# openfheorg/openfhe-development

Measured on AMD Instinct MI355X. Metric: NTT GB/s vs HBM roofline + CKKS EvalMultKeySwitch/sec, N=2^16 L=30, 1/2/4/8 GPU, higher is better.
Workload: dtype u64; 1 GPU; batched fwd+inv negacyclic NTT, N=2^16, L=30 x 60-bit limbs, 1024 polynomials per GPU (BASELINE configs[1]); global_batch=1024, parallelism=batch-sharded x1, no data-path collective

## Files before the change

openfhe-development_amd/csrc/fhe_hip.cpp:

```cpp
#include "../../include/fhe_hip.h"

#include <algorithm>
#include <cmath>
#include <cstdio>
#include <cstdlib>
#include <map>
#include <mutex>
#include <shared_mutex>
#include <string>
#include <type_traits>
#include <vector>

#include "basis_kernels.h"
#include "bfv_kernels.h"
#include "elemwise_kernels.h"
#include "host_math.h"
#include "ntt_kernels.h"
#include "ntt_static.h"
#include "ntt_row8.h"
#include "rt.h"
#include "sampler_kernels.h"
#include "blake2_kernels.h"

using namespace fhe;

static thread_local std::string g_lastError;
static fhe_status fail(fhe_status code, const std::string& msg) {
    g_lastError = msg;
    return code;
}
#define RT_CHECK(expr)                                                                  \
    do {                                                                                \
        const char* _e = (expr);                                                        \
        if (_e)                                                                         \
            return fail(FHE_ERR_DEVICE, std::string(#expr) + ": " + _e);                \
    } while (0)
#define ARG_CHECK(cond, msg)                  \
    do {                                      \
        if (!(cond))                          \
            return fail(FHE_ERR_ARG, msg);    \
    } while (0)

extern "C" const char* fhe_last_error(void) { return g_lastError.c_str(); }
extern "C" const char* fhe_version(void) {
#ifdef FHE_EMU
    return "fhe_hip 0.1 (TEST lane emulator build — not a product build)";
#else
    return "fhe_hip 0.1 (gfx950)";
#endif
}
extern "C" int fhe_device_count(void) { return rt::device_count(); }

namespace fhe {
namespace host {
bool is_prime(uint64_t n) {
    static const uint64_t w[] = {2, 3, 5, 7, 11, 13, 17, 19, 23, 29, 31, 37};
    if (n < 2)
        return false;
    for (uint64_t p : w) {
        if (n == p)
            return true;
        if (n % p == 0)
            return false;
    }
    uint64_t d = n - 1;
    int s      = 0;
    while (!(d & 1)) {
        d >>= 1;
        ++s;
    }
    for (uint64_t a : w) {
        uint64_t x = powmod(a, d, n);
        if (x == 1 || x == n - 1)
            continue;
        bool comp = true;
        for (int r = 1; r < s && comp; ++r) {
            x = mulmod(x, x, n);
            if (x == n - 1)
                comp = false;
        }
        if (comp)
            return false;
    }
    return true;
}
bool is_primitive_root_2n(uint64_t psi, uint64_t twoN, uint64_t q) {
    return psi != 0 && psi < q && powmod(psi, twoN / 2, q) == q - 1;
}
uint64_t first_prime(uint32_t bits, uint64_t m) {
    uint64_t q = (uint64_t)1 << bits, r = q % m, c = q + 1 - r;
    if (r > 0)
        c += m;
    while (!is_prime(c))
        c += m;
    return c;
}
uint64_t last_prime(uint32_t bits, uint64_t m) {
// ... 328 lines not shown
extern "C" fhe_status fhe_event_create(fhe_ctx* c, void** event) {
    ARG_CHECK(c && event, "fhe_event_create: null argument");
    RT_CHECK(rt::set_device(c->device));
    rt::event_t e;
    RT_CHECK(rt::event_create(&e));
    *event = (void*)e;
    return FHE_OK;
}
extern "C" fhe_status fhe_event_record(fhe_ctx* c, void* event, void* stream) {
    ARG_CHECK(c && event, "fhe_event_record: null argument");
    RT_CHECK(rt::set_device(c->device));
    RT_CHECK(rt::event_record((rt::event_t)event, (rt::stream_t)stream));
    return FHE_OK;
}
extern "C" fhe_status fhe_stream_wait_event(fhe_ctx* c, void* stream, void* event) {
    ARG_CHECK(c && event, "fhe_stream_wait_event: null argument");
    RT_CHECK(rt::set_device(c->device));
    RT_CHECK(rt::stream_wait_event((rt::stream_t)stream, (rt::event_t)event));
    return FHE_OK;
}
extern "C" fhe_status fhe_event_destroy(fhe_ctx* c, void* event) {
    ARG_CHECK(c, "fhe_event_destroy: null context");
    if (event)
        RT_CHECK(rt::event_destroy((rt::event_t)event));
    return FHE_OK;
}
extern "C" fhe_status fhe_memset_zero(fhe_ctx* c, void* dst, size_t bytes, void* stream) {
    ARG_CHECK(c && dst, "fhe_memset_zero: null argument");
    RT_CHECK(rt::set_device(c->device));
    RT_CHECK(rt::dzero(dst, bytes, (rt::stream_t)stream));
    return FHE_OK;
}
extern "C" fhe_status fhe_graph_begin(fhe_ctx* c, void* stream) {
    ARG_CHECK(c && stream, "fhe_graph_begin: capture needs a stream created with fhe_stream_create");
    RT_CHECK(rt::set_device(c->device));
    RT_CHECK(rt::capture_begin((rt::stream_t)stream));
    return FHE_OK;
}
extern "C" fhe_status fhe_graph_end(fhe_ctx* c, void* stream, void** graph) {
    ARG_CHECK(c && stream && graph, "fhe_graph_end: null argument");
    rt::graph_t g;
    RT_CHECK(rt::capture_end((rt::stream_t)stream, &g));
    *graph = (void*)g;
    return FHE_OK;
}
extern "C" fhe_status fhe_graph_launch(fhe_ctx* c, void* graph, void* stream) {
    ARG_CHECK(c && graph, "fhe_graph_launch: null argument");
    RT_CHECK(rt::graph_launch((rt::graph_t)graph, (rt::stream_t)stream));
    return FHE_OK;
}
extern "C" void fhe_graph_destroy(void* graph) {
    if (graph)
        rt::graph_destroy((rt::graph_t)graph);
}

static fhe_status make_sel(const fhe_ctx* c, const uint32_t* limbIdx, uint32_t nLimbs, LimbSel* sel, const char* who) {
    if (nLimbs < 1 || nLimbs > (uint32_t)kMaxLimbs)
        return fail(FHE_ERR_ARG, std::string(who) + ": nLimbs out of range");
    for (uint32_t i = 0; i < nLimbs; ++i) {
        uint32_t l = limbIdx ? limbIdx[i] : i;
        if (l >= c->L)
            return fail(FHE_ERR_ARG, std::string(who) + ": limb index exceeds context size");
        sel->idx[i] = (uint8_t)l;
    }
    for (uint32_t i = nLimbs; i < (uint32_t)kMaxLimbs; ++i)
        sel->idx[i] = 0;
    return FHE_OK;
}
static inline uint32_t tiles_for(const fhe_ctx* c, uint64_t rows) {
    const uint64_t words = rows << c->logN;
    return (uint32_t)((words + kTile - 1) >> kTileLog);
}
#define LAUNCH_CHECK() RT_CHECK(rt::last_launch_error())

static uint32_t env_u32(const char* name, uint32_t dflt) {
    const char* v = std::getenv(name);
    return v ? (uint32_t)std::strtoul(v, nullptr, 10) : dflt;
}
constexpr bool kHandoverDefault = true;
struct NttSwitches {
    int row8 = -1, row8X1 = -1;
    uint32_t row8Batch = 0, t1 = 0;
    bool handover = kHandoverDefault;
};
static const NttSwitches& ntt_switches() {
    static const NttSwitches sw = [] {
        NttSwitches s;
        auto flag = [](const char* name) {
            const char* v = std::getenv(name);
            return v && (v[0] == '0' || v[0] == '1') ? v[0] - '0' : -1;
        };
        s.row8   = flag("FHE_NTT_ROW8");
        s.row8X1 = flag("FHE_NTT_ROW8_X1");
        if (const char* v = std::getenv("FHE_NTT_ROW8_BATCH"))
            s.row8Batch = (v[0] == '1' || v[0] == '2' || v[0] == '4') && !v[1] ? (uint32_t)(v[0] - '0') : 0u;
        if (const char* v = std::getenv("FHE_NTT_HANDOVER")) {
            s.handover = v[0] == '1' && !v[1];
            if (!s.handover && !(v[0] == '0' && !v[1]))
                fprintf(stderr, "fhe_hip: FHE_NTT_HANDOVER=%s is neither 0 nor 1: hand-over is off\n", v);
        }
        s.t1 = env_u32("FHE_NTT_T1", 0);
        return s;
    }();
    return sw;
}
static bool row8_for(uint32_t T) { return ntt_switches().row8 >= 0 ? ntt_switches().row8 == 1 : T <= 11u; }
constexpr uint32_t kRow8BatchDefault = 2;
constexpr bool kRow8X1RegionsP2 = false, kRow8X1RegionsP4 = false;
static uint32_t row8_batch_for(uint32_t T) {
    if (T != 12u)
        return 1u;
    return ntt_switches().row8Batch ? ntt_switches().row8Batch : ntt_switches().row8 >= 0 ? 1u : kRow8BatchDefault;
}
static bool row8_x1_regions(uint32_t P) {
    return ntt_switches().row8X1 >= 0 ? ntt_switches().row8X1 == 1 : (P == 2 ? kRow8X1RegionsP2 : kRow8X1RegionsP4);
}
static uint32_t ntt_t1(uint32_t logN) {
    const uint32_t forced = ntt_switches().t1;
    if (forced >= 4 && forced <= 5 && logN > (uint32_t)kTileLog && logN - forced >= 9 && logN - forced <= 12)
        return forced;
    return std::max(4u, logN - (uint32_t)kTileLog);
}

struct NttPass {
    enum Kind { Single, Column, Row };
    bool inverse = false;
    Kind kind    = Single;
    uint32_t T   = 0;
    int mode = 1;
    NttPass() = default;
    NttPass(bool inv, Kind k, uint32_t stages) : inverse(inv), kind(k), T(stages), mode(k == Row ? (inv ? 0 : 9) : 1) {}
    bool layoutA() const { return kind == Column; }
};
struct NttPasses {
    uint32_t n;
    NttPass p[2];
};
static NttPasses ntt_passes(const fhe_ctx* c, bool inverse) {
    if (c->logN <= (uint32_t)kTileLog)
        return {1, {NttPass(inverse, NttPass::Single, c->logN), NttPass()}};
    const uint32_t T1 = ntt_t1(c->logN);
    const NttPass col(inverse, NttPass::Column, T1), row(inverse, NttPass::Row, c->logN - T1);
    return inverse ? NttPasses{2, {row, col}} : NttPasses{2, {col, row}};
}

struct NttEpilogue {
    uint32_t mode = 0, split = 0, aStride = 0, aFirst = 0;
    int64_t aDelta = 0;
    const uint64_t* A = nullptr;
    const TwPair* C   = nullptr;
    uint64_t *out0 = nullptr, *out1 = nullptr;
};
struct NttView {
    uint32_t stride = 0;
    uint32_t first  = 0;
};
struct NttOpts {
    NttView src, dst;
    int64_t srcDelta = 0;
    const NttEpilogue* epi = nullptr;
    bool canonOut = true;
    const uint32_t* proSrcLimb = nullptr;
    const TwPair* proC = nullptr;
    uint32_t proRows = 0;
};

static void plan_pass(bool inverse, bool layoutA, NttPassArgs& a) {
    const uint32_t logN = a.logN, T = a.T;
    const int logC  = kTileLog - (int)T;
    const int jsh   = layoutA ? (int)(logN - T) : 0;
    const int ish   = layoutA ? logC : 0;
    const int nst   = (int)(T + 3) / 4;
    int sizes[4];
    for (int i = 0; i < nst; ++i)
        sizes[i] = (int)T / nst + (i < (int)T % nst ? 1 : 0);
    NttStep real[4] = {};
// ... 798 lines not shown
    a.out = out, a.q = c->d_q, a.logN = c->logN, a.nLimbs = nl, a.batch = bt, a.seed = seed, a.stream = streamId, a.kind = kind;
    a.cdf = nullptr, a.cdfLen = 0, a.a = 0.0;
    if (kind == 1)
        if (fhe_status s = dgg_table(c, sigma, &a.cdf, &a.cdfLen, &a.a, who))
            return s;
    const uint64_t lanes = kind == 0 ? ((uint64_t)bt * nl) << c->logN : (uint64_t)bt << c->logN;
    FHE_LAUNCH(sample_kernel, (uint32_t)((lanes + kThreads - 1) / kThreads), st, a);
    LAUNCH_CHECK();
    return FHE_OK;
}
extern "C" fhe_status fhe_sample_uniform(fhe_ctx* c, uint64_t* out, const uint32_t* li, uint32_t nl, uint32_t bt, uint64_t seed,
                                         uint32_t streamId, void* st) {
    return sample_run(c, out, li, nl, bt, 0, 0.0, seed, streamId, st, "fhe_sample_uniform");
}
extern "C" fhe_status fhe_sample_gaussian(fhe_ctx* c, uint64_t* out, const uint32_t* li, uint32_t nl, uint32_t bt, double sigma,
                                          uint64_t seed, uint32_t streamId, void* st) {
    return sample_run(c, out, li, nl, bt, 1, sigma, seed, streamId, st, "fhe_sample_gaussian");
}
extern "C" fhe_status fhe_sample_ternary(fhe_ctx* c, uint64_t* out, const uint32_t* li, uint32_t nl, uint32_t bt, uint64_t seed,
                                         uint32_t streamId, void* st) {
    return sample_run(c, out, li, nl, bt, 2, 0.0, seed, streamId, st, "fhe_sample_ternary");
}

template <int KIND>
static fhe_status blake2_launch(const fhe_ctx* c, Blake2Args& a, const uint32_t* key, uint64_t counter0, void* st) {
    for (int i = 0; i < 16; ++i)
        a.key[i] = key[i];
    a.counter0 = counter0;
    const uint64_t minWaves = 8ull * (c->cus ? c->cus : 256);
    a.walk = kB2MaxWalk;
    while (a.walk > 1 && a.nBlocks / a.walk < minWaves)
        a.walk >>= 1;
    const uint64_t perWg = (uint64_t)(kB2Threads / 64) * a.walk;
    if (a.nBlocks)
        FHE_LAUNCH_BARRIER_N(blake2xb_kernel<KIND>, (a.nBlocks + perWg - 1) / perWg, kB2Threads, st, a);
    for (int i = 0; i < 16; ++i)
        ((volatile uint32_t*)a.key)[i] = 0;
    LAUNCH_CHECK();
    return FHE_OK;
}
extern "C" fhe_status fhe_blake2xb_stream(fhe_ctx* c, uint32_t* out, uint64_t nBlocks, const uint32_t key[16], uint64_t counter0, void* st) {
    ARG_CHECK(c && key && (out || nBlocks == 0), "fhe_blake2xb_stream: null argument");
    ARG_CHECK(((uintptr_t)out & 7u) == 0, "fhe_blake2xb_stream: out must be 8-byte aligned");
    ARG_CHECK(nBlocks <= ((uint64_t)UINT32_MAX - 1) * 4, "fhe_blake2xb_stream: nBlocks too large for one launch");
    RT_CHECK(rt::set_device(c->device));
    Blake2Args a{};
    a.out = (uint64_t*)out, a.nBlocks = nBlocks;
    return blake2_launch<3>(c, a, key, counter0, st);
}
static fhe_status blake2_sample(fhe_ctx* c, uint64_t* out, const uint32_t* li, uint32_t nl, uint32_t bt, int kind, double sigma,
                                const uint32_t* key, uint64_t counter0, void* st, const char* who) {
    ARG_CHECK(c && out && key && bt >= 1, std::string(who) + ": null argument or empty batch");
    Blake2Args a{};
    if (fhe_status s = make_sel(c, li, nl, &a.sel, who))
        return s;
    RT_CHECK(rt::set_device(c->device));
    a.out = out, a.q = c->d_q, a.mu128 = c->d_mu128, a.logN = c->logN, a.nLimbs = nl;
    if (kind == 1)
        if (fhe_status s = dgg_table(c, sigma, &a.cdf, &a.cdfLen, &a.a, who))
            return s;
    a.total   = kind == 0 ? ((uint64_t)bt * nl) << c->logN : (uint64_t)bt << c->logN;
    a.nBlocks = kind == 0 ? (a.total + 255) / 256 : (a.total + 511) / 512;
    return kind == 0   ? blake2_launch<0>(c, a, key, counter0, st)
           : kind == 1 ? blake2_launch<1>(c, a, key, counter0, st)
                       : blake2_launch<2>(c, a, key, counter0, st);
}
extern "C" fhe_status fhe_sample_uniform_blake2(fhe_ctx* c, uint64_t* out, const uint32_t* li, uint32_t nl, uint32_t bt,
                                                const uint32_t key[16], uint64_t counter0, void* st) {
    return blake2_sample(c, out, li, nl, bt, 0, 0.0, key, counter0, st, "fhe_sample_uniform_blake2");
}
extern "C" fhe_status fhe_sample_gaussian_blake2(fhe_ctx* c, uint64_t* out, const uint32_t* li, uint32_t nl, uint32_t bt, double sigma,
                                                 const uint32_t key[16], uint64_t counter0, void* st) {
    return blake2_sample(c, out, li, nl, bt, 1, sigma, key, counter0, st, "fhe_sample_gaussian_blake2");
}
extern "C" fhe_status fhe_sample_ternary_blake2(fhe_ctx* c, uint64_t* out, const uint32_t* li, uint32_t nl, uint32_t bt,
                                                const uint32_t key[16], uint64_t counter0, void* st) {
    return blake2_sample(c, out, li, nl, bt, 2, 0.0, key, counter0, st, "fhe_sample_ternary_blake2");
}

struct fhe_conv {
    fhe_ctx* ctx;
    uint32_t nSrc, nDst;
    std::vector<uint32_t> srcIdx, dstIdx;
    ConvTables tb;
    std::vector<ConvTables> chunks;
    const TwPair* allHatInv  = nullptr;
    const uint64_t* allSrcQ  = nullptr;
    const double* allQInv    = nullptr;
    std::vector<void*> owned;
};

static uint32_t conv_nsrc_pad(uint32_t nSrc) { return nSrc <= 8 ? 8u : nSrc <= 16 ? 16u : 32u; }
static fhe_status conv_from_tables(fhe_ctx* c, const std::vector<uint64_t>& src, const std::vector<uint64_t>& dst,
                                   const uint64_t* hatInvIn, const uint64_t* hatModIn, const uint64_t* alphaIn,
                                   const double* qInvIn, fhe_conv** out) {
    const uint32_t nSrc = (uint32_t)src.size(), nDst = (uint32_t)dst.size();
    if (nSrc < 1 || nSrc > (uint32_t)kMaxLimbs || nDst < 1 || nDst > (uint32_t)kMaxLimbs)
        return fail(FHE_ERR_ARG, "basis conversion: 1..256 source and target limbs");
    fhe_conv* cv = new fhe_conv;
    cv->ctx      = c;
    cv->nSrc     = nSrc;
    cv->nDst     = nDst;
    std::vector<uint64_t> mu(2 * (size_t)nDst), alphaMod((size_t)(nSrc + 1) * nDst, 0), red(4 * (size_t)nDst);
    for (uint32_t j = 0; j < nDst; ++j) {
        host::mu128(dst[j], &mu[2 * j]);
        const uint64_t R = (uint64_t)((((unsigned __int128)1) << 64) % dst[j]);
        red[4 * j]       = dst[j];
        red[4 * j + 1]   = R;
        red[4 * j + 2]   = host::shoup(R, dst[j]);
        red[4 * j + 3]   = (uint64_t)((((unsigned __int128)1) << 64) / dst[j]);
    }
    if (alphaIn)
        for (size_t k = 0; k < alphaMod.size(); ++k)
            alphaMod[k] = alphaIn[k] % dst[k % nDst];
    ConvTables shared{};
    fhe_status s;
    if ((s = dev_copy(&cv->owned, dst.data(), dst.size(), &shared.dstQ)) ||
        (s = dev_copy(&cv->owned, mu.data(), mu.size(), &shared.dstMu)) ||
        (s = dev_copy(&cv->owned, red.data(), red.size(), &shared.dstRed)) ||
        (s = dev_copy(&cv->owned, alphaMod.data(), alphaMod.size(), &shared.alphaMod))) {
        fhe_conv_destroy(cv);
        return s;
    }
    for (uint32_t c0 = 0; c0 < nSrc; c0 += 32u) {
        const uint32_t n   = std::min(32u, nSrc - c0);
        const uint32_t pad = conv_nsrc_pad(n);
        std::vector<TwPair> hatInv(32, TwPair{0, 0});
        std::vector<uint64_t> hatMod((size_t)pad * nDst, 0), srcPad(32, 1);
        std::vector<double> qInv(32, 0.0);
        for (uint32_t i = 0; i < n; ++i) {
            const uint64_t inv = hatInvIn[c0 + i] % src[c0 + i];
            hatInv[i]          = TwPair{inv, host::shoup(inv, src[c0 + i])};
            qInv[i]            = qInvIn ? qInvIn[c0 + i] : 1.0 / static_cast<double>(src[c0 + i]);
            srcPad[i]          = src[c0 + i];
            for (uint32_t j = 0; j < nDst; ++j)
                hatMod[(size_t)j * pad + i] = hatModIn[(size_t)(c0 + i) * nDst + j] % dst[j];
        }
        ConvTables tb = shared;
        if ((s = dev_copy(&cv->owned, hatInv.data(), hatInv.size(), &tb.hatInv)) ||
            (s = dev_copy(&cv->owned, hatMod.data(), hatMod.size(), &tb.hatMod)) ||
            (s = dev_copy(&cv->owned, srcPad.data(), srcPad.size(), &tb.srcQ)) ||
            (s = dev_copy(&cv->owned, qInv.data(), qInv.size(), &tb.srcQInv))) {
            fhe_conv_destroy(cv);
            return s;
        }
        cv->chunks.push_back(tb);
    }
    cv->tb = cv->chunks[0];
    if (nSrc > 32u) {
        std::vector<TwPair> allInv(nSrc);
        std::vector<double> allQInv(nSrc);
        for (uint32_t i = 0; i < nSrc; ++i) {
            const uint64_t inv = hatInvIn[i] % src[i];
            allInv[i]          = TwPair{inv, host::shoup(inv, src[i])};
            allQInv[i]         = qInvIn ? qInvIn[i] : 1.0 / static_cast<double>(src[i]);
        }
        if ((s = dev_copy(&cv->owned, allInv.data(), allInv.size(), &cv->allHatInv)) ||
            (s = dev_copy(&cv->owned, src.data(), src.size(), &cv->allSrcQ)) ||
            (s = dev_copy(&cv->owned, allQInv.data(), allQInv.size(), &cv->allQInv))) {
            fhe_conv_destroy(cv);
            return s;
        }
    }
    *out = cv;
    return FHE_OK;
}
static fhe_status conv_build(fhe_ctx* c, const std::vector<uint64_t>& src, const std::vector<uint64_t>& dst, fhe_conv** out,
                             const uint64_t* srcScale = nullptr, const uint64_t* dstScale = nullptr) {
    const uint32_t nSrc = (uint32_t)src.size(), nDst = (uint32_t)dst.size();
    std::vector<uint64_t> hatInv(nSrc), hatMod((size_t)nSrc * nDst), alphaMod((size_t)(nSrc + 1) * nDst);
    for (uint32_t i = 0; i < nSrc; ++i) {
        const uint64_t hat = host::prod_mod(src, (int)i, src[i]);
        hatInv[i]          = host::invmod(hat, src[i]);
        if (srcScale)
            hatInv[i] = host::mulmod(hatInv[i], srcScale[i] % src[i], src[i]);
        for (uint32_t j = 0; j < nDst; ++j) {
            uint64_t v = host::prod_mod(src, (int)i, dst[j]);
            if (dstScale)
                v = host::mulmod(v, dstScale[j] % dst[j], dst[j]);
            hatMod[(size_t)i * nDst + j] = v;
        }
    }
    for (uint32_t j = 0; j < nDst; ++j) {
        const uint64_t Qmod = host::prod_mod(src, -1, dst[j]);
        for (uint32_t a = 0; a <= nSrc; ++a)
// ... 31 lines not shown
    std::vector<uint64_t> src(nSrc), dst(nDst);
    for (uint32_t i = 0; i < nSrc; ++i) {
        ARG_CHECK(srcIdx[i] < c->L, "fhe_conv_create_custom: source limb exceeds context size");
        src[i] = c->q[srcIdx[i]];
    }
    for (uint32_t j = 0; j < nDst; ++j) {
        ARG_CHECK(dstIdx[j] < c->L, "fhe_conv_create_custom: target limb exceeds context size");
        dst[j] = c->q[dstIdx[j]];
    }
    RT_CHECK(rt::set_device(c->device));
    if (fhe_status s = conv_from_tables(c, src, dst, hatInv, hatMod, alphaMod, qInv, out))
        return s;
    (*out)->srcIdx.assign(srcIdx, srcIdx + nSrc);
    (*out)->dstIdx.assign(dstIdx, dstIdx + nDst);
    return FHE_OK;
}
extern "C" void fhe_conv_destroy(fhe_conv* cv) {
    if (!cv)
        return;
    for (void* p : cv->owned)
        rt::dfree(p);
    delete cv;
}

template <bool EXACT>
static fhe_status conv_run(fhe_conv* cv, const uint64_t* in, uint32_t inStride, uint32_t inFirst, uint64_t* out,
                           uint32_t outStride, uint32_t outFirst, uint32_t batch, void* st) {
    ARG_CHECK(cv && in && out, "fhe_switch_basis: null argument");
    ARG_CHECK(batch >= 1 && inFirst + cv->nSrc <= inStride && outFirst + cv->nDst <= outStride,
              "fhe_switch_basis: limb window exceeds tower stride");
    RT_CHECK(rt::set_device(cv->ctx->device));
    ConvArgs g{};
    g.in = in, g.out = out, g.tb = cv->tb;
    g.logN = cv->ctx->logN, g.batch = batch, g.nSrc = cv->nSrc, g.nDst = cv->nDst;
    g.inStride = inStride, g.inFirst = inFirst, g.outStride = outStride, g.outFirst = outFirst;
    const uint64_t coeffs = (uint64_t)batch << g.logN;
    const uint32_t grid   = (uint32_t)((coeffs + kThreads - 1) / kThreads);
    static const bool split30 = env_u32("FHE_CONV_SUM8", 2) != 1u;
    if (cv->chunks.size() > 1) {
        g.nSrcAll = cv->nSrc, g.inAll = in + ((size_t)inFirst << g.logN);
        g.allHatInv = cv->allHatInv, g.allSrcQ = cv->allSrcQ, g.allQInv = cv->allQInv;
        for (size_t k = 0; k < cv->chunks.size(); ++k) {
            g.tb      = cv->chunks[k];
            g.nSrc    = std::min(32u, cv->nSrc - 32u * (uint32_t)k);
            g.inFirst = inFirst + 32u * (uint32_t)k;
            g.acc     = k > 0;
            g.last    = k + 1 == cv->chunks.size();
            const uint32_t pad = conv_nsrc_pad(g.nSrc);
            if (pad == 8)
                FHE_LAUNCH((switch_basis_kernel<8, EXACT, 2, true>), grid, st, g);
            else if (pad == 16)
                FHE_LAUNCH((switch_basis_kernel<16, EXACT, 2, true>), grid, st, g);
            else
                FHE_LAUNCH((switch_basis_kernel<32, EXACT, 2, true>), grid, st, g);
            LAUNCH_CHECK();
        }
        return FHE_OK;
    }
    const uint32_t pad = conv_nsrc_pad(cv->nSrc);
    if (pad == 8 && split30)
        FHE_LAUNCH((switch_basis_kernel<8, EXACT, 2>), grid, st, g);
    else if (pad == 8)
        FHE_LAUNCH((switch_basis_kernel<8, EXACT, 1>), grid, st, g);
    else if (pad == 16 && split30)
        FHE_LAUNCH((switch_basis_kernel<16, EXACT, 2>), grid, st, g);
    else if (pad == 16)
        FHE_LAUNCH((switch_basis_kernel<16, EXACT, 1>), grid, st, g);
    else if (split30)
        FHE_LAUNCH((switch_basis_kernel<32, EXACT, 2>), grid, st, g);
    else
        FHE_LAUNCH((switch_basis_kernel<32, EXACT, 1>), grid, st, g);
    LAUNCH_CHECK();
    return FHE_OK;
}
extern "C" fhe_status fhe_approx_switch_basis(fhe_conv* cv, const uint64_t* in, uint32_t is, uint32_t ifst,
                                              uint64_t* out, uint32_t os, uint32_t ofst, uint32_t b, void* st) {
    return conv_run<false>(cv, in, is, ifst, out, os, ofst, b, st);
}
extern "C" fhe_status fhe_switch_basis_exact(fhe_conv* cv, const uint64_t* in, uint32_t is, uint32_t ifst,
                                             uint64_t* out, uint32_t os, uint32_t ofst, uint32_t b, void* st) {
    return conv_run<true>(cv, in, is, ifst, out, os, ofst, b, st);
}

extern "C" size_t fhe_expand_crt_basis_workspace_bytes(const fhe_conv* cv, uint32_t batch) {
    return cv ? (((size_t)batch * cv->nSrc) << cv->ctx->logN) * 8 : 0;
}
static fhe_status expand_run(fhe_conv* cv, const uint64_t* x, int inEval, uint64_t* out, int resultEval, int reverseOrder,
                             uint32_t batch, void* ws, size_t wsBytes, void* st, bool exact) {
    ARG_CHECK(cv && x && out && batch >= 1, "fhe_expand_crt_basis: bad argument");
    ARG_CHECK(!cv->srcIdx.empty(), "fhe_expand_crt_basis: the plan must come from fhe_conv_create[_custom]");
    fhe_ctx* c = cv->ctx;
    RT_CHECK(rt::set_device(c->device));
    const uint32_t nQ = cv->nSrc, nP = cv->nDst, tot = nQ + nP;
    const uint32_t qFirst = reverseOrder ? nP : 0, pFirst = reverseOrder ? 0 : nQ;
    const size_t rowB = (size_t)8 << c->logN;
    const uint64_t* coef = x;
    if (inEval) {
        ARG_CHECK(ws && wsBytes >= fhe_expand_crt_basis_workspace_bytes(cv, batch), "fhe_expand_crt_basis: workspace too small");
        if (fhe_status s = ntt_run(c, true, x, (uint64_t*)ws, cv->srcIdx.data(), nQ, batch, st))
            return s;
        coef = (const uint64_t*)ws;
    }
    if (fhe_status s = exact ? conv_run<true>(cv, coef, nQ, 0, out, tot, pFirst, batch, st)
                             : conv_run<false>(cv, coef, nQ, 0, out, tot, pFirst, batch, st))
        return s;
    const uint64_t* qsrc = (resultEval && inEval) ? x : coef;
    uint64_t* qdst       = out + ((size_t)qFirst << c->logN);
    RT_CHECK(rt::d2d_2d(qdst, tot * rowB, qsrc, nQ * rowB, nQ * rowB, batch, (rt::stream_t)st));
    if (resultEval) {
        NttOpts rows;
        rows.src.stride = rows.dst.stride = tot;
        rows.src.first = rows.dst.first = qFirst;
        if (!inEval)
            if (fhe_status s = ntt_run(c, false, out, out, cv->srcIdx.data(), nQ, batch, st, rows))
                return s;
        rows.src.first = rows.dst.first = pFirst;
        return ntt_run(c, false, out, out, cv->dstIdx.data(), nP, batch, st, rows);
    }
    return FHE_OK;
}
extern "C" fhe_status fhe_expand_crt_basis(fhe_conv* cv, const uint64_t* x, int inEval, uint64_t* out, int resultEval,
                                           int reverseOrder, uint32_t batch, void* ws, size_t wsBytes, void* st) {
    return expand_run(cv, x, inEval, out, resultEval, reverseOrder, batch, ws, wsBytes, st, true);
}
extern "C" fhe_status fhe_mod_up(fhe_conv* cv, const uint64_t* x, int inEval, uint64_t* out, uint32_t batch, void* ws,
                                 size_t wsBytes, void* st) {
    return expand_run(cv, x, inEval, out, 1, 0, batch, ws, wsBytes, st, false);
}
extern "C" fhe_status fhe_fast_expand_crt_basis_p_over_q(fhe_conv* toPl, fhe_conv* toQl, const uint64_t* x, uint64_t* out,
                                                         uint32_t batch, void* st) {
    ARG_CHECK(toPl && toQl && x && out && batch >= 1, "fhe_fast_expand_crt_basis_p_over_q: bad argument");
    ARG_CHECK(toQl->nSrc == toPl->nDst, "fhe_fast_expand_crt_basis_p_over_q: the second plan must start from the first plan's target basis");
    const uint32_t nQl = toQl->nDst, nPl = toPl->nDst, tot = nQl + nPl;
    if (fhe_status s = conv_run<false>(toPl, x, toPl->nSrc, 0, out, tot, nQl, batch, st))
        return s;
    return conv_run<true>(toQl, out, tot, nQl, out, tot, 0, batch, st);
}

struct fhe_ks_plan {
    fhe_ctx* ctx;
    uint32_t sizeQ, sizeP, numPartQ, alpha;
    struct Level {
        uint32_t sizeQl = 0, numParts = 0;
        std::vector<fhe_conv*> up;
        std::vector<std::vector<uint32_t>> cidx;
        std::vector<uint32_t> partSize;
        fhe_conv* down = nullptr;
        std::map<uint64_t, fhe_conv*> downT;
        TwPair* d_PInv = nullptr;
        TwPair* d_PModq = nullptr;
    };
    std::vector<Level*> levels;
    std::vector<void*> owned;
    std::map<std::vector<uint64_t>, void*> bsgsTables;
    uint64_t* d_zeroRows = nullptr;
    std::mutex cacheMutex;
};
struct fhe_ks_key {
    fhe_ks_plan* plan;
    uint64_t *d_b = nullptr, *d_a = nullptr;
    size_t words = 0;
    bool owned = true;
};

extern "C" fhe_status fhe_ks_plan_create(fhe_ctx* c, uint32_t sizeQ, uint32_t sizeP, uint32_t numPartQ,
                                         fhe_ks_plan** out) {
    ARG_CHECK(c && out, "fhe_ks_plan_create: null argument");
    ARG_CHECK(sizeQ >= 1 && sizeP >= 1 && sizeQ + sizeP <= c->L, "fhe_ks_plan_create: context must hold Q then P limbs");
    ARG_CHECK(numPartQ >= 1, "numPartQ is zero");
    const uint32_t a = (sizeQ + numPartQ - 1) / numPartQ;
    ARG_CHECK(sizeQ > a * (numPartQ - 1),
              "HYBRID key switching parameters: Can't appropriately distribute towers into digits");
    fhe_ks_plan* p = new fhe_ks_plan;
    p->ctx = c, p->sizeQ = sizeQ, p->sizeP = sizeP, p->numPartQ = numPartQ, p->alpha = a;
    p->levels.assign(sizeQ + 1, nullptr);
    *out = p;
    return FHE_OK;
}
static void ks_level_free(fhe_ks_plan::Level* lv) {
    if (!lv)
        return;
    for (auto* cv : lv->up)
        fhe_conv_destroy(cv);
    fhe_conv_destroy(lv->down);
    for (auto& kv : lv->downT)
        fhe_conv_destroy(kv.second);
    delete lv;
}
extern "C" void fhe_ks_plan_destroy(fhe_ks_plan* p) {
    if (!p)
        return;
    for (auto* lv : p->levels)
        ks_level_free(lv);
    for (void* q : p->owned)
        rt::dfree(q);
    for (auto& kv : p->bsgsTables)
        rt::dfree(kv.second);
    delete p;
// ... 69 lines not shown
        fhe_ks_key_destroy(k);
        return fail(FHE_ERR_ALLOC, "fhe_ks_key_alloc: device allocation failed");
    }
    *out = k;
    return FHE_OK;
}
extern "C" fhe_status fhe_ks_key_upload(fhe_ks_plan* p, const uint64_t* keyB, const uint64_t* keyA, fhe_ks_key** out) {
    ARG_CHECK(keyB && keyA, "fhe_ks_key_upload: null key");
    fhe_ks_key* k = nullptr;
    if (fhe_status s = fhe_ks_key_alloc(p, &k))
        return s;
    RT_CHECK(rt::h2d(k->d_b, keyB, k->words * 8, nullptr));
    RT_CHECK(rt::h2d(k->d_a, keyA, k->words * 8, nullptr));
    RT_CHECK(rt::sync(nullptr));
    *out = k;
    return FHE_OK;
}
extern "C" fhe_status fhe_ks_key_wrap(fhe_ks_plan* p, uint64_t* devB, uint64_t* devA, fhe_ks_key** out) {
    ARG_CHECK(p && devB && devA && out, "fhe_ks_key_wrap: null argument");
    fhe_ks_key* k = new fhe_ks_key;
    k->plan       = p;
    k->words      = (size_t)p->numPartQ * (p->sizeQ + p->sizeP) << p->ctx->logN;
    k->d_b        = devB;
    k->d_a        = devA;
    k->owned      = false;
    *out          = k;
    return FHE_OK;
}
extern "C" void fhe_ks_key_destroy(fhe_ks_key* k) {
    if (!k)
        return;
    if (k->owned && k->d_b)
        rt::dfree(k->d_b);
    if (k->owned && k->d_a)
        rt::dfree(k->d_a);
    delete k;
}
extern "C" uint64_t* fhe_ks_key_devptr(fhe_ks_key* k, int which) { return k ? (which ? k->d_a : k->d_b) : nullptr; }
extern "C" size_t fhe_ks_key_words(const fhe_ks_key* k) { return k ? k->words : 0; }

struct KsLayout {
    size_t coef = 0, e0 = 0, e1 = 0, md = 0, pcoef = 0, d2 = 0, k0 = 0, k1 = 0, total = 0;
    std::vector<size_t> dig;
};
static KsLayout ks_layout(const fhe_ks_plan* p, uint32_t sizeQl, uint32_t batch) {
    KsLayout w;
    const size_t N = (size_t)1 << p->ctx->logN;
    const uint32_t numParts = std::min((sizeQl + p->alpha - 1) / p->alpha, p->numPartQ);
    w.dig.assign(numParts, 0);
    size_t off = 0;
    w.coef = off, off += (size_t)batch * sizeQl * N;
    for (uint32_t j = 0; j < numParts; ++j) {
        const uint32_t start = p->alpha * j;
        const uint32_t sz    = (j == numParts - 1) ? sizeQl - start : p->alpha;
        w.dig[j] = off, off += (size_t)batch * (sizeQl - sz + p->sizeP) * N;
    }
    w.e0 = off, off += (size_t)batch * (sizeQl + p->sizeP) * N;
    w.e1 = off, off += (size_t)batch * (sizeQl + p->sizeP) * N;
    w.md = off, off += (size_t)2 * batch * sizeQl * N;
    w.pcoef = off, off += (size_t)2 * batch * p->sizeP * N;
    w.d2 = off, off += (size_t)batch * sizeQl * N;
    w.k0 = off, off += (size_t)batch * sizeQl * N;
    w.k1 = off, off += (size_t)batch * sizeQl * N;
    w.total = off;
    return w;
}
extern "C" size_t fhe_ks_workspace_bytes(const fhe_ks_plan* p, uint32_t sizeQl, uint32_t batch) {
    if (!p || sizeQl < 1 || sizeQl > p->sizeQ || batch < 1)
        return 0;
    return ks_layout(p, sizeQl, batch).total * 8;
}

static fhe_status mod_down_core(fhe_ks_plan* p, fhe_ks_plan::Level* lv, const uint64_t* x, uint32_t nTow, uint64_t* pcoef,
                                uint64_t* md, void* st, fhe_conv* down = nullptr, const NttEpilogue* epi = nullptr) {
    fhe_ctx* c            = p->ctx;
    const uint32_t sizeQl = lv->sizeQl, sizeP = p->sizeP, sizeQlP = sizeQl + sizeP;
    std::vector<uint32_t> pIdx(sizeP);
    for (uint32_t j = 0; j < sizeP; ++j)
        pIdx[j] = p->sizeQ + j;
    NttOpts pRows;
    pRows.src.stride = sizeQlP, pRows.src.first = sizeQl;
    if (fhe_status s = ntt_run(c, true, x, pcoef, pIdx.data(), sizeP, nTow, st, pRows))
        return s;
    if (fhe_status s = fhe_approx_switch_basis(down ? down : lv->down, pcoef, sizeP, 0, md, sizeQl, 0, nTow, st))
        return s;
    NttOpts fused;
    fused.epi = epi;
    return ntt_run(c, false, md, md, nullptr, sizeQl, nTow, st, fused);
}
static fhe_status mod_down_tail(fhe_ks_plan* p, fhe_ks_plan::Level* lv, const uint64_t* x, const uint64_t* md, uint32_t nTow,
                                uint64_t* out, bool accumulate, void* st) {
    const uint32_t sizeQl = lv->sizeQl, sizeQlP = sizeQl + p->sizeP;
    if (accumulate)
        return elem_run<OP_SUB_MUL_CONST_ACC>(p->ctx, out, x, md, lv->d_PInv, nullptr, sizeQl, nTow, st, "fhe_approx_mod_down",
                                              sizeQlP, 0);
    return elem_run<OP_SUB_MUL_CONST>(p->ctx, out, x, md, lv->d_PInv, nullptr, sizeQl, nTow, st, "fhe_approx_mod_down", sizeQlP, 0);
}
static fhe_status mod_down_run(fhe_ks_plan* p, fhe_ks_plan::Level* lv, const uint64_t* x, uint32_t nTow, uint64_t* out,
                               uint64_t* pcoef, uint64_t* md, void* st) {
    if (fhe_status s = mod_down_core(p, lv, x, nTow, pcoef, md, st))
        return s;
    return mod_down_tail(p, lv, x, md, nTow, out, false, st);
}

static fhe_status ks_precompute_run(fhe_ks_plan* p, fhe_ks_plan::Level* lv, const uint64_t* cin, uint32_t batch,
                                    uint64_t* ws, const KsLayout& w, void* st) {
    fhe_ctx* c            = p->ctx;
    const uint32_t sizeQl = lv->sizeQl;
    if (fhe_status s = fhe_ntt_inv_oop(c, cin, ws + w.coef, nullptr, sizeQl, batch, st))
        return s;
    NttOpts lazy;
    lazy.canonOut = false;
    for (uint32_t j = 0; j < lv->numParts; ++j) {
        const uint32_t nc = (uint32_t)lv->cidx[j].size();
        uint64_t* dj      = ws + w.dig[j];
        if (fhe_status s = fhe_approx_switch_basis(lv->up[j], ws + w.coef, sizeQl, p->alpha * j, dj, nc, 0, batch, st))
            return s;
        if (fhe_status s = ntt_run(c, false, dj, dj, lv->cidx[j].data(), nc, batch, st, lazy))
            return s;
    }
    return FHE_OK;
}
static fhe_status ks_inner_multi_launch(fhe_ks_plan* p, fhe_ks_plan::Level* lv, const fhe_ks_key* const* keys, uint32_t nKeys,
                                        const uint64_t* cin, uint32_t batch, uint64_t* const* e0, uint64_t* const* e1,
                                        const uint64_t* first, const TwPair* dP, uint64_t* ws, const KsLayout& w, void* st,
                                        uint32_t towOff = 0) {
    fhe_ctx* c            = p->ctx;
    const uint32_t sizeQl = lv->sizeQl, sizeP = p->sizeP, sizeQlP = sizeQl + sizeP;
    const uint32_t tilesPerRow = c->N >= (uint32_t)kTile ? (c->N >> kTileLog) : 1u;
    for (uint32_t t0 = 0; t0 < nKeys; t0 += (uint32_t)kMaxMultiKeys) {
        KsInnerMultiArgs g;
        const uint32_t nt = std::min<uint32_t>(kMaxMultiKeys, nKeys - t0);
        for (uint32_t j = 0; j < (uint32_t)kMaxDigits; ++j) {
            g.nc[j]     = j < lv->numParts ? (uint32_t)lv->cidx[j].size() : 0u;
            g.digits[j] = j < lv->numParts ? ws + w.dig[j] + (((size_t)towOff * g.nc[j]) << c->logN) : nullptr;
        }
        for (uint32_t t = 0; t < (uint32_t)kMaxMultiKeys; ++t) {
            const uint32_t tt = t < nt ? t0 + t : t0;
            g.keyB[t] = keys[tt]->d_b, g.keyA[t] = keys[tt]->d_a, g.out0[t] = e0[tt], g.out1[t] = e1[tt];
        }
        g.c = cin + (((size_t)towOff * sizeQl) << c->logN), g.first = first, g.firstC = dP;
        g.lc = c->d_lc, g.mu128 = c->d_mu128, g.red = c->d_red;
        g.logN = c->logN, g.batch = batch, g.sizeQl = sizeQl, g.sizeQ = p->sizeQ, g.sizeP = sizeP;
        g.numDigits = lv->numParts, g.alpha = p->alpha, g.nKeys = nt;
        const uint64_t grid = (((uint64_t)tilesPerRow * sizeQlP + 7) / 8) * 8 * batch;
        static const uint32_t ksm = env_u32("FHE_KSM", 1);
        uintptr_t bits = (uintptr_t)g.c | (uintptr_t)g.first;
        for (uint32_t j = 0; j < lv->numParts && j < (uint32_t)kMaxDigits; ++j)
            bits |= (uintptr_t)g.digits[j];
        for (uint32_t t = 0; t < nt; ++t)
            bits |= (uintptr_t)g.keyB[t] | (uintptr_t)g.keyA[t] | (uintptr_t)g.out0[t] | (uintptr_t)g.out1[t];
        const bool wide = (bits & 15u) == 0 && c->N >= 2;
        if (lv->numParts <= 3 && ksm == 1 && wide)
            FHE_LAUNCH((ks_inner_multi_kernel<3, 2, true>), grid, st, g);
        else if (lv->numParts <= 3 && ksm == 2 && wide)
            FHE_LAUNCH((ks_inner_multi_kernel<3, 2, false>), grid, st, g);
        else if (lv->numParts <= 3 && ksm == 3)
            FHE_LAUNCH((ks_inner_multi_kernel<3, 1, false>), grid, st, g);
        else if (lv->numParts <= 3)
            FHE_LAUNCH((ks_inner_multi_kernel<3>), grid, st, g);
        else if (lv->numParts <= 4)
            FHE_LAUNCH((ks_inner_multi_kernel<4>), grid, st, g);
        else
            FHE_LAUNCH((ks_inner_multi_kernel<8>), grid, st, g);
        LAUNCH_CHECK();
    }
    return FHE_OK;
}
static fhe_status ks_inner_run(fhe_ks_plan* p, fhe_ks_plan::Level* lv, const fhe_ks_key* key, const uint64_t* cin,
                               uint32_t batch, uint64_t* e0, uint64_t* e1, uint64_t* ws, const KsLayout& w, void* st,
                               uint32_t towOff = 0) {
    fhe_ctx* c            = p->ctx;
    const uint32_t sizeQl = lv->sizeQl, sizeP = p->sizeP, sizeQlP = sizeQl + sizeP;
    const uint32_t tilesPerRow = c->N >= (uint32_t)kTile ? (c->N >> kTileLog) : 1u;
    if (lv->numParts <= (uint32_t)kMaxDigits)
        return ks_inner_multi_launch(p, lv, &key, 1, cin, batch, &e0, &e1, nullptr, nullptr, ws, w, st, towOff);
    for (uint32_t j0 = 0; j0 < lv->numParts; j0 += (uint32_t)kMaxDigits) {
        KsInnerArgs g;
        const uint32_t nd = std::min<uint32_t>(kMaxDigits, lv->numParts - j0);
        for (uint32_t j = 0; j < (uint32_t)kMaxDigits; ++j) {
            g.nc[j]     = j < nd ? (uint32_t)lv->cidx[j0 + j].size() : 0u;
            g.digits[j] = j < nd ? ws + w.dig[j0 + j] + (((size_t)towOff * g.nc[j]) << c->logN) : nullptr;
        }
        g.c = cin + (((size_t)towOff * sizeQl) << c->logN), g.keyB = key->d_b, g.keyA = key->d_a;
        g.out0 = e0, g.out1 = e1;
        g.lc = c->d_lc, g.mu128 = c->d_mu128, g.red = c->d_red;
        g.logN = c->logN, g.batch = batch, g.sizeQl = sizeQl, g.sizeQ = p->sizeQ, g.sizeP = sizeP;
        g.numDigits = nd, g.alpha = p->alpha, g.j0 = j0, g.acc = j0 > 0;
        FHE_LAUNCH(ks_inner_product_kernel, (((uint64_t)tilesPerRow * sizeQlP + 7) / 8) * 8 * batch, st, g);
        LAUNCH_CHECK();
    }
    return FHE_OK;
}
static fhe_status ks_inner_multi_run(fhe_ks_plan* p, fhe_ks_plan::Level* lv, const fhe_ks_key* const* keys, uint32_t nKeys,
                                     const uint64_t* cin, uint32_t batch, uint64_t* const* e0, uint64_t* const* e1,
                                     const uint64_t* first, const TwPair* dP, uint64_t* ws, const KsLayout& w, void* st) {
    if (lv->numParts <= (uint32_t)kMaxDigits)
        return ks_inner_multi_launch(p, lv, keys, nKeys, cin, batch, e0, e1, first, dP, ws, w, st);
    const uint32_t sizeQl = lv->sizeQl, sizeQlP = sizeQl + p->sizeP;
    for (uint32_t t = 0; t < nKeys; ++t) {
        if (fhe_status s = ks_inner_run(p, lv, keys[t], cin, batch, e0[t], e1[t], ws, w, st))
// ... 2770 lines not shown
```

Measured before the change: 2354 GB/s.

## Fuse approximate basis conversion with the first forward NTT column pass

Adds a conv_column kernel that performs the approximate CRT basis conversion for small source counts (up to 8 limbs) and applies the first 4-stage NTT column pass in registers before writing, then runs only the second NTT pass. It is wired into mod-down, key-switch digit precompute and CRT expansion. This removes one full write-and-read round trip of the converted limbs through HBM. The cost is more LDS and register pressure per block, plus a fallback path that is used when the NTT plan shape or moduli do not match. The metric is the standalone NTT, which this change likely does not touch.

```diff
diff --git a/openfhe-development_amd/csrc/conv_column.h b/openfhe-development_amd/csrc/conv_column.h
--- /dev/null
+++ b/openfhe-development_amd/csrc/conv_column.h
@@ -0,0 +1,137 @@
+#ifndef FHE_CONV_COLUMN_H
+#define FHE_CONV_COLUMN_H
+#include "basis_kernels.h"
+#include "ntt_static.h"
+
+namespace fhe {
+
+constexpr int kConvColMaxSrc = 8;
+struct ConvColumnArgs {
+    const uint64_t* in;
+    uint64_t* out;
+    ConvTables tb;
+    const TwPair* tw;
+    const uint64_t* q;
+    const uint64_t* red;
+    uint32_t logN, batch, nSrc, nDst;
+    uint32_t inStride, inFirst, outStride, outFirst;
+    uint32_t xcdSwizzle;
+    LimbSel sel;
+};
+
+FHE_HD uint64_t pack30(uint64_t y) {
+    uint32_t y0, y1;
+    split30(y, y0, y1);
+    return (uint64_t)y0 | ((uint64_t)y1 << 32);
+}
+
+template <int C, int NT, int NS>
+FHE_DEV void conv_column_targets(const ConvColumnArgs& g, const uint64_t* lds, uint32_t b, uint32_t jbase) {
+    constexpr int HALVES = C / 64, NW = NT / 64;
+    const uint32_t t = FHE_TID, logN = g.logN;
+    const uint32_t S = (1u << logN) >> 4;
+    const uint32_t wave = FHE_UNIFORM(t >> 6), lane = t & 63u;
+    BflyZero z{0, 0};
+#ifdef FHE_PINNED_ASM
+    asm volatile("v_mov_b32 %0, 0\n\tv_mov_b32 %1, 0" : "={v65}"(z.z0), "={v81}"(z.z1));
+#endif
+    for (uint32_t u = wave; u < g.nDst * (uint32_t)HALVES; u += (uint32_t)NW) {
+        const uint32_t j = u / (uint32_t)HALVES, cl = (u % (uint32_t)HALVES) * 64u + lane;
+        uint32_t h0[NS], h1[NS];
+#pragma unroll
+        for (int k = 0; k < NS; ++k)
+            split30(FHE_ULOAD64(g.tb.hatMod, (uint64_t)j * kConvColMaxSrc + k), h0[k], h1[k]);
+        const uint64_t p    = FHE_ULOAD64(g.tb.dstQ, j);
+        const uint64_t mulo = FHE_ULOAD64(g.tb.dstMu, 2 * j), muhi = FHE_ULOAD64(g.tb.dstMu, 2 * j + 1);
+        const uint32_t kp   = 64u - (uint32_t)__builtin_clzll(p);
+        uint64_t r[16];
+        const uint64_t* Y = lds + cl;
+#pragma unroll
+        for (int row = 0; row < 16; ++row) {
+            sum8s s8;
+            sum8s_clear(s8);
+#pragma unroll
+            for (int k = 0; k < NS; ++k) {
+                const uint64_t y = Y[(k * 16 + row) * C];
+                sum8s_add(s8, (uint32_t)y, (uint32_t)(y >> 32), h0[k], h1[k]);
+            }
+            r[row] = sum8s_reduce(s8, p, kp, mulo, muhi);
+        }
+        const uint32_t limb = FHE_UNIFORM(g.sel.idx[j]);
+        const uint64_t q    = FHE_ULOAD64(g.q, limb);
+        FHE_BOUND_CHECK(q == p, "conv_column: the target's modulus is not its context limb's");
+        const uint64_t twoq = q << 1, nq = 0 - q;
+        const uint64_t redc = FHE_ULOAD64(g.red, limb);
+        const BflyConst c{(uint32_t)nq, (uint32_t)(nq >> 32), q, twoq, 0 - twoq, twoq + q, (uint32_t)redc, (uint32_t)(redc >> 32)};
+        TwSrc ts;
+        ts.tw         = g.tw + ((uint64_t)limb << logN);
+        ts.rowLane    = nullptr;
+        ts.fin        = nullptr;
+        ts.shared     = nullptr;
+        ts.sharedLane = 0;
+        using P = SPlan<true, false, 4>;
+        static_assert(P::nst == 1 && !P::sweep(0, 1), "the 4-stage column pass is one step on canonical input");
+        run_step<true, false, 4, 0, false, false>(r, ts, jbase + cl, logN, c, z, 1u);
+        run_red16(r, c);
+        uint64_t* dst = g.out + (((uint64_t)b * g.outStride + g.outFirst + j) << logN) + jbase + cl;
+#pragma unroll
+        for (int row = 0; row < 16; ++row) {
+            *dst = r[row];
+            dst += S;
+#if defined(__HIP_DEVICE_COMPILE__)
+            asm volatile("" : "+v"(dst));
+#endif
+        }
+    }
+}
+
+template <int C, int NT, int NS>
+FHE_GLOBAL void FHE_LAUNCH_BOUNDS(NT) conv_column_kernel(const ConvColumnArgs g) {
+    static_assert(C % 64 == 0 && NT % C == 0 && 16 % (NT / C) == 0, "whole waves per row segment, whole sweeps per limb");
+    static_assert(NS >= 1 && NS <= kConvColMaxSrc, "one sum8s chunk");
+    FHE_SHARED_U64(lds, NS * 16 * C);
+    const uint32_t t = FHE_TID, logN = g.logN;
+    const uint32_t S = (1u << logN) >> 4;
+    const uint32_t tilesPerTower = S / (uint32_t)C;
+    uint32_t b, tile;
+    if (g.xcdSwizzle) {
+        const uint32_t xcd = FHE_BID & 7u, i = FHE_BID >> 3;
+        b    = i % g.batch;
+        tile = (i / g.batch) * 8u + xcd;
+    }
+    else {
+        b    = FHE_BID / tilesPerTower;
+        tile = FHE_BID % tilesPerTower;
+    }
+    const uint32_t jbase = tile * (uint32_t)C;
+
+    constexpr int RS  = NT / C;
+    constexpr int RPT = 16 / RS;
+    constexpr int KB  = 16 / RPT > 8 ? 8 : 16 / RPT;
+    const uint32_t col = t % (uint32_t)C, r0 = t / (uint32_t)C;
+    const uint64_t* in = g.in + (((uint64_t)b * g.inStride + g.inFirst) << logN) + jbase + col;
+    const uint64_t* hp = reinterpret_cast<const uint64_t*>(g.tb.hatInv);
+#pragma unroll
+    for (int k0 = 0; k0 < NS; k0 += KB) {
+        uint64_t x[KB][RPT];
+#pragma unroll
+        for (int kk = 0; kk < KB && k0 + kk < NS; ++kk)
+#pragma unroll
+            for (int i = 0; i < RPT; ++i)
+                x[kk][i] = in[((uint64_t)(k0 + kk) << logN) + (uint64_t)(r0 + (uint32_t)(i * RS)) * S];
+#pragma unroll
+        for (int kk = 0; kk < KB && k0 + kk < NS; ++kk) {
+            const uint32_t k = (uint32_t)(k0 + kk);
+            const uint64_t w = FHE_ULOAD64(hp, 2 * k), wp = FHE_ULOAD64(hp, 2 * k + 1), qk = FHE_ULOAD64(g.tb.srcQ, k);
+#pragma unroll
+            for (int i = 0; i < RPT; ++i)
+                lds[(k * 16u + r0 + (uint32_t)(i * RS)) * (uint32_t)C + col] = pack30(mul_shoup(x[kk][i], w, wp, qk));
+        }
+    }
+    FHE_SYNC();
+
+    conv_column_targets<C, NT, NS>(g, lds, b, jbase);
+}
+
+}
+#endif
diff --git a/openfhe-development_amd/csrc/fhe_hip.cpp b/openfhe-development_amd/csrc/fhe_hip.cpp
--- a/openfhe-development_amd/csrc/fhe_hip.cpp
+++ b/openfhe-development_amd/csrc/fhe_hip.cpp
@@ -13,6 +13,7 @@
 
 #include "basis_kernels.h"
 #include "bfv_kernels.h"
+#include "conv_column.h"
 #include "elemwise_kernels.h"
 #include "host_math.h"
 #include "ntt_kernels.h"
@@ -507,6 +508,7 @@
     int row8 = -1, row8X1 = -1;
     uint32_t row8Batch = 0, t1 = 0;
     bool handover = kHandoverDefault;
+    int convFused = -1;
 };
 static const NttSwitches& ntt_switches() {
     static const NttSwitches sw = [] {
@@ -517,6 +519,7 @@
         };
         s.row8   = flag("FHE_NTT_ROW8");
         s.row8X1 = flag("FHE_NTT_ROW8_X1");
+        s.convFused = flag("FHE_CONV_FUSED");
         if (const char* v = std::getenv("FHE_NTT_ROW8_BATCH"))
             s.row8Batch = (v[0] == '1' || v[0] == '2' || v[0] == '4') && !v[1] ? (uint32_t)(v[0] - '0') : 0u;
         if (const char* v = std::getenv("FHE_NTT_HANDOVER")) {
@@ -1481,6 +1484,7 @@
     fhe_ctx* ctx;
     uint32_t nSrc, nDst;
     std::vector<uint32_t> srcIdx, dstIdx;
+    std::vector<uint64_t> dstMod;
     ConvTables tb;
     std::vector<ConvTables> chunks;
     const TwPair* allHatInv  = nullptr;
@@ -1500,6 +1504,7 @@
     cv->ctx      = c;
     cv->nSrc     = nSrc;
     cv->nDst     = nDst;
+    cv->dstMod   = dst;
     std::vector<uint64_t> mu(2 * (size_t)nDst), alphaMod((size_t)(nSrc + 1) * nDst, 0), red(4 * (size_t)nDst);
     for (uint32_t j = 0; j < nDst; ++j) {
         host::mu128(dst[j], &mu[2 * j]);
@@ -1697,6 +1702,60 @@
     return conv_run<true>(cv, in, is, ifst, out, os, ofst, b, st);
 }
 
+constexpr uint32_t kConvColCols = 64, kConvColThreads = 512;
+static bool conv_column_instance(const fhe_ctx* c, const fhe_conv* cv, const ConvColumnArgs* a, void* stream) {
+    const NttPasses f = ntt_passes(c, false);
+    if (!(f.n == 2 && f.p[0].T == 4 && f.p[0].mode == 1 && static_instance(f.p[0], nullptr, nullptr)))
+        return false;
+    if (!(cv->chunks.size() == 1 && cv->nSrc <= (uint32_t)kConvColMaxSrc && conv_nsrc_pad(cv->nSrc) == (uint32_t)kConvColMaxSrc))
+        return false;
+    if (a) {
+        const uint32_t grid = a->batch * ((c->N >> 4) / kConvColCols);
+        switch (cv->nSrc) {
+#define FHE_CASE(NS) \
+    case NS: FHE_LAUNCH_AS("", (conv_column_kernel<kConvColCols, kConvColThreads, NS>), grid, kConvColThreads, true, stream, *a); break;
+            FHE_CASE(1) FHE_CASE(2) FHE_CASE(3) FHE_CASE(4) FHE_CASE(5) FHE_CASE(6) FHE_CASE(7) FHE_CASE(8)
+#undef FHE_CASE
+        }
+    }
+    return true;
+}
+static fhe_status conv_ntt_fwd_run(fhe_ctx* c, fhe_conv* cv, const uint64_t* in, uint32_t inStride, uint32_t inFirst, uint64_t* out,
+                                   const uint32_t* dstIdx, uint32_t batch, void* st, const NttOpts& o, uint32_t outStride = 0,
+                                   uint32_t outFirst = 0) {
+    ARG_CHECK(cv && in && out && batch >= 1, "conversion + transform: bad argument");
+    const uint32_t nDst = cv->nDst;
+    bool fused = ntt_switches().convFused != 0 && conv_column_instance(c, cv, nullptr, nullptr) && !o.src.stride && !o.dst.stride &&
+                 !o.srcDelta && !o.proSrcLimb;
+    for (uint32_t j = 0; fused && j < nDst; ++j)
+        fused = (dstIdx ? dstIdx[j] : j) < c->L && c->q[dstIdx ? dstIdx[j] : j] == cv->dstMod[j];
+    NttOpts rows = o;
+    if (outStride)
+        rows.src.stride = rows.dst.stride = outStride, rows.src.first = rows.dst.first = outFirst;
+    if (!fused) {
+        if (fhe_status s = fhe_approx_switch_basis(cv, in, inStride, inFirst, out, outStride ? outStride : nDst, outFirst, batch, st))
+            return s;
+        return ntt_run(c, false, out, out, dstIdx, nDst, batch, st, rows);
+    }
+    ARG_CHECK(!outStride || outFirst + nDst <= outStride, "conversion + transform: limb window exceeds tower stride");
+    ARG_CHECK(inFirst + cv->nSrc <= inStride, "conversion + transform: limb window exceeds tower stride");
+    ConvColumnArgs g{};
+    if (fhe_status s = make_sel(c, dstIdx, nDst, &g.sel, "conversion + transform"))
+        return s;
+    RT_CHECK(rt::set_device(c->device));
+    g.in = in, g.out = out, g.tb = cv->tb;
+    g.tw = c->d_tw, g.q = c->d_q, g.red = c->d_red;
+    g.logN = c->logN, g.batch = batch, g.nSrc = cv->nSrc, g.nDst = nDst;
+    g.inStride = inStride, g.inFirst = inFirst, g.outStride = outStride ? outStride : nDst, g.outFirst = outStride ? outFirst : 0;
+    g.xcdSwizzle = ((c->N >> 4) / kConvColCols) % 8u == 0 ? 1u : 0u;
+    conv_column_instance(c, cv, &g, st);
+    LAUNCH_CHECK();
+    NttOpts second;
+    second.src = second.dst = rows.dst;
+    second.epi = o.epi, second.canonOut = o.canonOut;
+    return launch_pass(c, ntt_passes(c, false).p[1], out, out, g.sel, nDst, batch, st, second);
+}
+
 extern "C" size_t fhe_expand_crt_basis_workspace_bytes(const fhe_conv* cv, uint32_t batch) {
     return cv ? (((size_t)batch * cv->nSrc) << cv->ctx->logN) * 8 : 0;
 }
@@ -1716,8 +1775,10 @@
             return s;
         coef = (const uint64_t*)ws;
     }
-    if (fhe_status s = exact ? conv_run<true>(cv, coef, nQ, 0, out, tot, pFirst, batch, st)
-                             : conv_run<false>(cv, coef, nQ, 0, out, tot, pFirst, batch, st))
+    const bool convAndNtt = !exact && resultEval;
+    if (fhe_status s = exact        ? conv_run<true>(cv, coef, nQ, 0, out, tot, pFirst, batch, st)
+                       : convAndNtt ? conv_ntt_fwd_run(c, cv, coef, nQ, 0, out, cv->dstIdx.data(), batch, st, NttOpts(), tot, pFirst)
+                                    : conv_run<false>(cv, coef, nQ, 0, out, tot, pFirst, batch, st))
         return s;
     const uint64_t* qsrc = (resultEval && inEval) ? x : coef;
     uint64_t* qdst       = out + ((size_t)qFirst << c->logN);
@@ -1729,6 +1790,8 @@
         if (!inEval)
             if (fhe_status s = ntt_run(c, false, out, out, cv->srcIdx.data(), nQ, batch, st, rows))
                 return s;
+        if (convAndNtt)
+            return FHE_OK;
         rows.src.first = rows.dst.first = pFirst;
         return ntt_run(c, false, out, out, cv->dstIdx.data(), nP, batch, st, rows);
     }
@@ -1964,11 +2027,9 @@
     pRows.src.stride = sizeQlP, pRows.src.first = sizeQl;
     if (fhe_status s = ntt_run(c, true, x, pcoef, pIdx.data(), sizeP, nTow, st, pRows))
         return s;
-    if (fhe_status s = fhe_approx_switch_basis(down ? down : lv->down, pcoef, sizeP, 0, md, sizeQl, 0, nTow, st))
-        return s;
     NttOpts fused;
     fused.epi = epi;
-    return ntt_run(c, false, md, md, nullptr, sizeQl, nTow, st, fused);
+    return conv_ntt_fwd_run(c, down ? down : lv->down, pcoef, sizeP, 0, md, nullptr, nTow, st, fused);
 }
 static fhe_status mod_down_tail(fhe_ks_plan* p, fhe_ks_plan::Level* lv, const uint64_t* x, const uint64_t* md, uint32_t nTow,
                                 uint64_t* out, bool accumulate, void* st) {
@@ -1994,11 +2055,8 @@
     NttOpts lazy;
     lazy.canonOut = false;
     for (uint32_t j = 0; j < lv->numParts; ++j) {
-        const uint32_t nc = (uint32_t)lv->cidx[j].size();
-        uint64_t* dj      = ws + w.dig[j];
-        if (fhe_status s = fhe_approx_switch_basis(lv->up[j], ws + w.coef, sizeQl, p->alpha * j, dj, nc, 0, batch, st))
-            return s;
-        if (fhe_status s = ntt_run(c, false, dj, dj, lv->cidx[j].data(), nc, batch, st, lazy))
+        uint64_t* dj = ws + w.dig[j];
+        if (fhe_status s = conv_ntt_fwd_run(c, lv->up[j], ws + w.coef, sizeQl, p->alpha * j, dj, lv->cidx[j].data(), batch, st, lazy))
             return s;
     }
     return FHE_OK;
```

Result: no change. 2355 GB/s (median of 4 runs) (+0.0%).
